# mnastorg/PSI-GNN

Hardware: AMD Instinct MI355X
Metric: fixed-point edges/sec (E' x Broyden iterations/sec) on 1M-node Poisson mesh (higher is better)
Workload: dtype f32

## Files before the change

### psi-gnn_amd/csrc/solver.hip

```cpp
#include "vec_helpers.h"
#include <stdlib.h>
#include <math.h>
#include <algorithm>
#include <vector>

struct Status {
  int32_t n_iter;
  int32_t done;
  int32_t prot_break;
  int32_t stop_reason;
  int32_t lowest_step;
  int32_t cur;
  int32_t low;
  int32_t nxt;
  double lowest_rel, lowest_abs_at;
  double rel0;
  double abs0;
  int32_t lowest_step_abs;
  int32_t stop_abs;
  double s, beta;
};

#define PARTA_LD 32
#define RB 256
#define RA 8
struct psignn_broyden {
  const psignn_plan* plan = nullptr;
  int64_t M = 0;
  int seq_len = D;
  int thr = 0;
  int keep_trace = 0;
  int vec = 16;
  int nblk = 0, npart = 0;
  int vec_ax = 0, nblk_ax = 0;
  int jgroups = 1;
  float* jpart = nullptr;
  float *U = nullptr, *V = nullptr;
  float* xbuf = nullptr;
  float* gbuf[2] = {nullptr, nullptr};
  float *upd = nullptr, *fx = nullptr, *fwork = nullptr;
  float* lwork = nullptr;
  int64_t lwork_floats = 0;
  float* nrm_part = nullptr;
  float* part2 = nullptr;
  int uvu = 0;
  int vec_u = 0, nblk_u = 0, npart_u = 0;
  int u2d_kmax = 0, nblk4 = 0, a_ready = 0;
  int u2d_keep = 0, a_from = 0;
  int u2d_reg = 1;
  float* parta = nullptr;
  int nn_cap = 0;
  float *h0p = nullptr, *prbp = nullptr, *nrmp = nullptr;
  float* part = nullptr;
  int ldp = 0;
  int64_t pstride = 0;
  float* coef = nullptr;
  Status* st = nullptr;
  double *rel_trace = nullptr, *abs_trace = nullptr;
  Status* h_st = nullptr;
  size_t bytes = 0;
  int ext_iter = 0;
  int64_t ld = 0;
  int hist = 0;
  int stop_abs = 0;
  int64_t size_hint = 0;
  int plan_order = 1;
};

__global__ void k_init_status(Status* st, double* rel_trace, double* abs_trace, int thr, int stop_abs = 0) {
  if (threadIdx.x == 0 && blockIdx.x == 0) {
    st->abs0 = 0.0; st->lowest_step_abs = 0; st->stop_abs = stop_abs;
    st->n_iter = 0; st->done = 0; st->prot_break = 0; st->stop_reason = 0; st->lowest_step = 0;
    st->cur = 0; st->low = 0; st->nxt = 1;
    st->lowest_rel = 1e8; st->lowest_abs_at = 1e8; st->rel0 = 0.0; st->s = 0.0; st->beta = 0.0;
  }
  for (int i = blockIdx.x * blockDim.x + threadIdx.x; i < thr; i += gridDim.x * blockDim.x) {
    rel_trace[i] = 0.0;
    abs_trace[i] = 0.0;
  }
}

template <int VEC>
__global__ __launch_bounds__(TB) void k_begin(int64_t M, const float* __restrict__ x0, const float* __restrict__ fx0,
                                              float* __restrict__ xb, float* __restrict__ gx, float* __restrict__ upd) {
  int64_t e0 = elem0<VEC>();
  if (e0 >= M) return;
  float a[VEC], b[VEC];
  ldv<VEC>(x0, e0, M, a);
  ldv<VEC>(fx0, e0, M, b);
  stv<VEC>(xb, e0, M, a);
#pragma unroll
  for (int i = 0; i < VEC; ++i) b[i] -= a[i];
  stv<VEC>(gx, e0, M, b);
  stv<VEC>(upd, e0, M, b);
}

template <int VEC>
__device__ __forceinline__ void xnext_body(int64_t M, const Status* __restrict__ st, float* __restrict__ xb,
                                           const float* __restrict__ upd, float* __restrict__ copy_out) {
  if (st->done) return;
  int64_t e0 = elem0<VEC>();
  if (e0 >= M) return;
  const float* xc = xb + (int64_t)st->cur * M;
  float* xn = xb + (int64_t)st->nxt * M;
  float a[VEC], b[VEC];
  ldv<VEC>(xc, e0, M, a);
  ldv<VEC>(upd, e0, M, b);
#pragma unroll
  for (int i = 0; i < VEC; ++i) a[i] += b[i];
  stv<VEC>(xn, e0, M, a);
  if (copy_out) stv<VEC>(copy_out, e0, M, a);
}
template <int VEC>
__global__ __launch_bounds__(TB) void k_xnext(int64_t M, const Status* __restrict__ st, float* __restrict__ xb,
                                              const float* __restrict__ upd, float* __restrict__ copy_out) {
  xnext_body<VEC>(M, st, xb, upd, copy_out);
}

template <int VEC>
__global__ __launch_bounds__(TB) void k_xtrial(int64_t M, const Status* __restrict__ st, const float* __restrict__ xb,
                                               float* __restrict__ upd, float s, float* __restrict__ out, int commit) {
  if (st->done) return;
  int64_t e0 = elem0<VEC>();
  if (e0 >= M) return;
  const float* xc = xb + (int64_t)st->cur * M;
  float a[VEC], b[VEC];
  ldv<VEC>(xc, e0, M, a);
  ldv<VEC>(upd, e0, M, b);
#pragma unroll
  for (int i = 0; i < VEC; ++i) {
    b[i] *= s;
    a[i] += b[i];
// ... 644 lines not shown
#pragma unroll
        for (int q = 0; q < U2D_UNROLL; ++q) {
          const float cc = __builtin_bit_cast(float, __builtin_amdgcn_readlane(__builtin_bit_cast(int, cv), q));
          const float cb = __builtin_bit_cast(float, __builtin_amdgcn_readlane(__builtin_bit_cast(int, cv), 8 + q));
          a1[0] = fmaf(-cc, u[q].x, a1[0]); a1[1] = fmaf(-cc, u[q].y, a1[1]); a1[2] = fmaf(-cc, u[q].z, a1[2]); a1[3] = fmaf(-cc, u[q].w, a1[3]);
          a2[0] = fmaf(-cb, u[q].x, a2[0]); a2[1] = fmaf(-cb, u[q].y, a2[1]); a2[2] = fmaf(-cb, u[q].z, a2[2]); a2[3] = fmaf(-cb, u[q].w, a2[3]);
        }
      }
      for (; j < j_keep0; ++j) {
        const float cc = rfl(coef[thr + j]), cb = rfl(coef[2 * thr + j]);
        asm volatile("" : "+v"(off));
        const float4 u = ld4_so(U + (int64_t)j * ld, off);
        a1[0] = fmaf(-cc, u.x, a1[0]); a1[1] = fmaf(-cc, u.y, a1[1]); a1[2] = fmaf(-cc, u.z, a1[2]); a1[3] = fmaf(-cc, u.w, a1[3]);
        a2[0] = fmaf(-cb, u.x, a2[0]); a2[1] = fmaf(-cb, u.y, a2[1]); a2[2] = fmaf(-cb, u.z, a2[2]); a2[3] = fmaf(-cb, u.w, a2[3]);
      }
      switch (k - j_keep0) {
        U2R_CASE(KB - 8, false) U2R_CASE(KB - 7, false) U2R_CASE(KB - 6, false) U2R_CASE(KB - 5, false) U2R_CASE(KB - 4, false)
        U2R_CASE(KB - 3, false) U2R_CASE(KB - 2, false) U2R_CASE(KB - 1, false) U2R_CASE(KB, false)
        default: break;
      }
    }
#undef U2R_CASE
  } else {
    const bool in = e0 < M;
    float a1[4] = {0.f, 0.f, 0.f, 0.f}, a2[4] = {0.f, 0.f, 0.f, 0.f};
    if (in) {
      float dg[4];
      ldv<4>(upd, e0, M, a1);
      ldv<4>(dgv, e0, M, dg);
      ldv<4>(gv, e0, M, a2);
#pragma unroll
      for (int i = 0; i < 4; ++i) dg[i] = a2[i] - dg[i];
#pragma unroll
      for (int i = 0; i < 4; ++i) a1[i] = a1[i] + dg[i];
    }
    for (int j = 0; j < k; ++j) {
      float u[4] = {0.f, 0.f, 0.f, 0.f};
      const float cc = coef[thr + j], cb = coef[2 * thr + j];
      if (in) ldv<4>(U + (int64_t)j * ld, e0, M, u);
#pragma unroll
      for (int i = 0; i < 4; ++i) {
        a1[i] = fmaf(-cc, u[i], a1[i]);
        a2[i] = fmaf(-cb, u[i], a2[i]);
      }
    }
    if (in) {
      const float sv = (float)st->s, beta = (float)st->beta;
#pragma unroll
      for (int i = 0; i < 4; ++i) {
        float q = a1[i] / sv;
        q = (q != q) ? 0.f : q;
        a1[i] = q;
        a2[i] = fmaf(-q, beta, a2[i]);
      }
      stv<4>(U + (int64_t)k * ld, e0, M, a1);
      stv<4>(upd, e0, M, a2);
#pragma unroll
      for (int i = 0; i < 4; ++i)
        if (e0 + i >= M) a1[i] = a2[i] = 0.f;
    }
    for (int jj = j_keep0; jj <= k; ++jj) {
      float u[4] = {a1[0], a1[1], a1[2], a1[3]};
      if (jj < k) {
        u[0] = u[1] = u[2] = u[3] = 0.f;
        if (in) ldv<4>(U + (int64_t)jj * ld, e0, M, u);
      }
      float sa = fmaf(u[0], a2[0], fmaf(u[1], a2[1], fmaf(u[2], a2[2], u[3] * a2[3])));
      sa = wave_sum(sa);
      if (lead) ua[wv][jj - j_keep0] = sa;
    }
  }
  __syncthreads();
  if (tid <= k - j_keep0) part[(int64_t)blockIdx.x * PARTA_LD + tid] = (ua[0][tid] + ua[1][tid]) + (ua[2][tid] + ua[3][tid]);
}
template <int KB> struct U2RWaves { static constexpr int value = KB <= 8 ? 8 : KB <= 16 ? 5 : 4; };
template <int KB>
__global__ __launch_bounds__(TB, U2RWaves<KB>::value) void k_sweep_u2r(int64_t M, int k, const Status* __restrict__ st, float* __restrict__ U,
                                                                      float* __restrict__ upd, const float* __restrict__ dgv,
                                                                      const float* __restrict__ gv, const float* __restrict__ coef, int thr,
                                                                      float* __restrict__ part, int64_t ld, int j_keep0) {
  sweep_u2r_body<KB>(M, k, st, U, upd, dgv, gv, coef, thr, part, ld, j_keep0);
}

template <int VEC>
__device__ __forceinline__ void axpy_finish(int64_t M, int k, int64_t e0, float* av, float* a1, float* a2, const float* dg,
                                            const float* g, float* __restrict__ U, float* __restrict__ V,
                                            float* __restrict__ upd, float& p1, float& p2, int64_t ld) {
#pragma unroll
  for (int i = 0; i < VEC; ++i) {
    p1 = fmaf(av[i], dg[i], p1);
    av[i] = (av[i] != av[i]) ? 0.f : av[i];
    p2 = fmaf(av[i], g[i], p2);
  }
  stv<VEC>(V + (int64_t)k * ld, e0, M, av);
  stv<VEC>(U + (int64_t)k * ld, e0, M, a1);
  stv<VEC>(upd, e0, M, a2);
}

template <int VEC>
__device__ __forceinline__ void axpy_body(int64_t M, int k, const Status* __restrict__ st, float* __restrict__ U,
                                             float* __restrict__ V, float* __restrict__ upd ,
                                             const float* __restrict__ dgv, const float* __restrict__ gv,
                                             const float* __restrict__ coef, int thr, float* __restrict__ part, int npart,
                                             int jstride, float* __restrict__ jpart, int64_t ld, const bool split) {
  if (st->done) return;
  const int j0 = blockIdx.y * jstride, j1 = min(k, j0 + jstride);
  int64_t e0 = elem0<VEC>();
  float p1 = 0.f, p2 = 0.f;
  if (e0 < M) {
    float av[VEC], a1[VEC], a2[VEC], dg[VEC], g[VEC];
    if (!split) {
      ldv<VEC>(upd, e0, M, av);
      ldv<VEC>(dgv, e0, M, dg);
      ldv<VEC>(gv, e0, M, g);
#pragma unroll
      for (int i = 0; i < VEC; ++i) dg[i] = g[i] - dg[i];
#pragma unroll
      for (int i = 0; i < VEC; ++i) {
        a1[i] = av[i] + dg[i];
        a2[i] = g[i];
        av[i] = -av[i];
      }
    } else {
#pragma unroll
      for (int i = 0; i < VEC; ++i) av[i] = a1[i] = a2[i] = 0.f;
    }
    for (int j = j0; j < j1; ++j) {
      float u[VEC], v[VEC];
      float ca = coef[j], cc = coef[thr + j], cb = coef[2 * thr + j];
      ldv_stream<VEC>(U + (int64_t)j * ld, e0, M, u);
      ldv_stream<VEC>(V + (int64_t)j * ld, e0, M, v);
#pragma unroll
      for (int i = 0; i < VEC; ++i) {
        av[i] = fmaf(ca, v[i], av[i]);
        a1[i] = fmaf(-cc, u[i], a1[i]);
        a2[i] = fmaf(-cb, u[i], a2[i]);
      }
    }
    if (split) {
      float* base = jpart + (int64_t)blockIdx.y * 3 * M;
      stv<VEC>(base, e0, M, av);
      stv<VEC>(base + M, e0, M, a1);
      stv<VEC>(base + 2 * M, e0, M, a2);
      return;
    }
    axpy_finish<VEC>(M, k, e0, av, a1, a2, dg, g, U, V, upd, p1, p2, ld);
  }
  if (split) return;
  block_pair_store(p1, p2, part, npart);
}
template <int VEC>
__global__ __launch_bounds__(TB) void k_axpy(int64_t M, int k, const Status* __restrict__ st, float* __restrict__ U,
                                             float* __restrict__ V, float* __restrict__ upd ,
                                             const float* __restrict__ dgv, const float* __restrict__ gv,
                                             const float* __restrict__ coef, int thr, float* __restrict__ part, int npart,
                                             int jstride, float* __restrict__ jpart, int64_t ld) {
  axpy_body<VEC>(M, k, st, U, V, upd, dgv, gv, coef, thr, part, npart, jstride, jpart, ld, gridDim.y > 1);
}

template <int VEC>
__device__ __forceinline__ void axpy_combine_body(int64_t M, int k, int G, const Status* __restrict__ st,
                                                     const float* __restrict__ jpart, float* __restrict__ U,
                                                     float* __restrict__ V, float* __restrict__ upd,
                                                     const float* __restrict__ dgv, const float* __restrict__ gv,
                                                     float* __restrict__ part, int npart, int64_t ld) {
  if (st->done) return;
// ... 74 lines not shown

template <int VEC>
__global__ __launch_bounds__(TB) void k_copy_sel(int64_t M, const float* __restrict__ xb, const int32_t* __restrict__ sel,
                                                 int fixed, float* __restrict__ dst) {
  int64_t e0 = elem0<VEC>();
  if (e0 >= M) return;
  int idx = sel ? *sel : fixed;
  float a[VEC];
  ldv<VEC>(xb + (int64_t)idx * M, e0, M, a);
  stv<VEC>(dst, e0, M, a);
}

int psignn_f_eval_p(const psignn_plan_t* p, const float* W, int nl, const float* hbase, const int32_t* d_sel,
                    int64_t stride, const float* h0, const float* prb, const float* nrm, float* out, float* work,
                    hipStream_t st);

int psignn_f_tile_fused(const psignn_plan* p, const float* W, int nl, float* xbuf, int64_t M, const int32_t* st_words,
                        int off_done, int off_cur, int off_nxt, const float* upd, float* gnew,
                        const float* h0, const float* prb, const float* nrm, float* part, hipStream_t st);

#define U2R_KB_MAX 24
#define U2D_LDS_KMAX (PARTA_LD - 1)
static_assert(U2R_KB_MAX + 1 <= PARTA_LD, "the register fold's kept pairs must fit a partials row");
__global__ __launch_bounds__(TB) void kb_sweep_u2d(const BatchDesc* __restrict__ descs, int k, int j_keep0, int par);
static bool u2d_lds_attr(int dev) {
  static int state[64] = {0};
  if (dev < 0 || dev >= 64) return false;
  if (state[dev] == 0) {
    const int want = U2D_LDS_KMAX * TB * 16;
    const bool ok = hipFuncSetAttribute((const void*)k_sweep_u2d, hipFuncAttributeMaxDynamicSharedMemorySize, want) == hipSuccess &&
                    hipFuncSetAttribute((const void*)kb_sweep_u2d, hipFuncAttributeMaxDynamicSharedMemorySize, want) == hipSuccess;
    if (!ok) (void)hipGetLastError();
    state[dev] = ok ? 1 : -1;
  }
  return state[dev] > 0;
}

static int broyden_alloc(psignn_broyden* s) {
  size_t M = (size_t)s->M, thr = (size_t)s->thr;
  const int64_t vec16_min = [] {
    const char* e = getenv("PSIGNN_VEC16_MIN");
    return e ? (int64_t)atoll(e) : (int64_t)3 << 18;
  }();
  const int64_t eff = std::max<int64_t>(s->M, s->size_hint);
  s->vec = eff >= vec16_min ? 16 : 4;
  s->nblk = (int)cdiv(s->M, (int64_t)s->vec * TB);
  const int64_t eff_blk = cdiv(eff, (int64_t)s->vec * TB);
  s->jgroups = eff_blk >= 768 ? 1 : (int)std::min<int64_t>(8, cdiv(768, eff_blk));
  const bool short_shard = s->size_hint > s->M && s->vec == 16 && s->nblk < 512;
  if (short_shard) s->jgroups = 4;
  if (const char* e = getenv("PSIGNN_JGROUPS")) s->jgroups = std::max(1, std::min(8, atoi(e)));
  s->npart = s->nblk * (TB / 64);
  s->vec_ax = s->vec;
  s->nblk_ax = s->nblk;
  const char* e_ax = getenv("PSIGNN_VEC_AX4");
  if (e_ax ? (atoi(e_ax) != 0 && s->vec == 16)
           : (s->vec == 16 && s->jgroups > 1 && (short_shard || cdiv(s->M, (int64_t)4 * TB) >= 512))) {
    s->vec_ax = 4;
    s->nblk_ax = (int)cdiv(s->M, (int64_t)4 * TB);
  }
  s->uvu = 0;
  if (s->vec == 16 && s->jgroups == 1 && s->vec_ax == 16) {
    s->uvu = 1; s->vec_u = 16; s->nblk_u = s->nblk;
  } else if (s->vec_ax == 4 && s->vec == 16) {
    s->uvu = 1; s->vec_u = 4; s->nblk_u = s->nblk_ax;
  }
  if (const char* e = getenv("PSIGNN_UVU")) if (atoi(e) == 0) s->uvu = 0;
  if (s->hist) {
    s->uvu = 1;
    s->vec_u = (s->vec == 16 && s->jgroups == 1 && s->vec_ax == 16) ? 16 : 4;
    s->nblk_u = (int)cdiv(s->M, (int64_t)s->vec_u * TB);
  }
  s->npart_u = s->nblk_u * (TB / 64);
  s->nblk4 = (int)cdiv(s->M, (int64_t)4 * TB);
  const bool fold_ok = s->uvu != 0;
  s->u2d_reg = cdiv(eff, (int64_t)4 * TB) >= 2048 && s->M < ((int64_t)1 << 30);
  if (const char* e = getenv("PSIGNN_U2D_FORM")) s->u2d_reg = ((e[0] == 'l' || e[0] == 'L') ? 0 : 1) && s->M < ((int64_t)1 << 30);
  const int kmax_cap = s->u2d_reg ? U2R_KB_MAX : U2D_LDS_KMAX;
  s->u2d_kmax = fold_ok ? 24 : 0;
  if (const char* e = getenv("PSIGNN_U2D_KMAX")) s->u2d_kmax = fold_ok ? std::max(0, std::min(kmax_cap, atoi(e))) : 0;
  s->u2d_keep = s->u2d_kmax > 0 ? 16 : 0;
  if (const char* e = getenv("PSIGNN_U2D_KEEP")) s->u2d_keep = s->u2d_kmax > 0 ? std::max(0, std::min(s->u2d_kmax, atoi(e))) : 0;
  if (s->hist) s->u2d_kmax = s->u2d_keep = 0;
  if (s->u2d_kmax > 0 && !s->u2d_reg) {
    int dev = 0;
    (void)hipGetDevice(&dev);
    if (!u2d_lds_attr(dev)) {
      s->u2d_kmax = std::min(s->u2d_kmax, 15);
      s->u2d_keep = std::min(s->u2d_keep, 15);
    }
  }
  s->nn_cap = std::max<int>(std::max(s->nblk, s->nblk_ax), s->plan ? (int)s->plan->n_tiles : 0);
  s->ldp = (s->thr + 63) / 64 * 64;
  s->pstride = (int64_t)std::max(std::max(s->nblk, s->nblk_u), std::max(s->nblk_ax, 1)) * s->ldp;
  size_t nx = s->keep_trace ? thr + 2 : 3;
  s->ld = s->hist ? (s->M + 127) / 128 * 128 : (s->M + 63) / 64 * 64;
  size_t ld = (size_t)s->ld;
  const size_t pb = s->hist ? 2 : 4;
  struct { void** p; size_t n; } allocs[] = {
      {(void**)&s->U, thr * ld * pb},  {(void**)&s->V, thr * ld * pb},   {(void**)&s->xbuf, nx * M * 4},
      {(void**)&s->gbuf[0], M * 4},   {(void**)&s->gbuf[1], M * 4},   {(void**)&s->upd, M * 4},
      {(void**)&s->fx, M * 4},        {(void**)&s->part, 3 * (size_t)s->pstride * 4 + 16}, {(void**)&s->parta, (size_t)s->nblk4 * PARTA_LD * 4 + 16},
      {(void**)&s->coef, (3 + RA) * thr * 4 + 16}, {(void**)&s->st, sizeof(Status)},
      {(void**)&s->nrm_part, 2 * (size_t)s->nn_cap * 4 + 16}, {(void**)&s->part2, 2 * (size_t)std::max(s->nblk, s->nblk_u) * 4 + 16},
      {(void**)&s->rel_trace, thr * 8 + 8}, {(void**)&s->abs_trace, thr * 8 + 8}};
  for (auto& a : allocs) {
    if (hipMalloc(a.p, a.n ? a.n : 16) != hipSuccess) {
      psignn_set_error("broyden: hipMalloc of %zu bytes failed (U+V need 2*thr*N*d*4 bytes)", a.n);
      return PSIGNN_ENOMEM;
    }
    s->bytes += a.n;
  }
  if (s->jgroups > 1 && s->vec_ax == s->vec) {
    size_t jb = (size_t)s->jgroups * 3 * M * 4;
    if (hipMalloc((void**)&s->jpart, jb) != hipSuccess) {
      psignn_set_error("broyden: hipMalloc of the split-sweep scratch failed");
      return PSIGNN_ENOMEM;
    }
    s->bytes += jb;
  }
  if (s->plan) {
    size_t wf = (size_t)psignn_f_workspace_floats(s->plan) * 4;
    if (hipMalloc((void**)&s->fwork, wf) != hipSuccess) {
      psignn_set_error("broyden: hipMalloc of f workspace failed");
      return PSIGNN_ENOMEM;
    }
    s->bytes += wf;
    size_t N = (size_t)s->plan->N;
    if (hipMalloc((void**)&s->h0p, M * 4) != hipSuccess || hipMalloc((void**)&s->prbp, N * 3 * 4) != hipSuccess ||
        hipMalloc((void**)&s->nrmp, N * 2 * 4) != hipSuccess) {
      psignn_set_error("broyden: hipMalloc of plan-order inputs failed");
      return PSIGNN_ENOMEM;
    }
    s->bytes += M * 4 + N * 20;
  }
  if (hipHostMalloc((void**)&s->h_st, sizeof(Status)) != hipSuccess) {
    psignn_set_error("broyden: hipHostMalloc failed");
    return PSIGNN_ENOMEM;
  }
  return 0;
}

extern "C" void psignn_broyden_destroy(psignn_broyden_t* s) {
  if (!s) return;
  void* ptrs[] = {s->U, s->V, s->xbuf, s->gbuf[0], s->gbuf[1], s->upd, s->fx, s->fwork, s->part, s->coef, s->st, s->nrm_part, s->part2, s->parta,
                  s->rel_trace, s->abs_trace, s->h0p, s->prbp, s->nrmp, s->jpart, s->lwork};
  for (void* q : ptrs)
    if (q) (void)hipFree(q);
  if (s->h_st) (void)hipHostFree(s->h_st);
  delete s;
}

extern "C" int psignn_broyden_create_opts(psignn_broyden_t** out, const psignn_plan_t* plan, int64_t n_elems, int seq_len, int threshold,
                                          int keep_trace, int64_t shard_elems, int history) {
  ARG_CHECK(out, "out is NULL");
  *out = nullptr;
  ARG_CHECK(history == 0 || history == 1, "history: 0 = fp32 pairs, 1 = bf16 pairs");
  if (plan) {
    ARG_CHECK(threshold > 0 && shard_elems >= 0, "bad arguments");
    ARG_CHECK((n_elems == 0 || n_elems == plan->N * D) && (seq_len == 0 || seq_len == D), "n_elems / seq_len do not match the plan");
  } else {
    ARG_CHECK(n_elems > 0 && threshold > 0 && seq_len > 0 && shard_elems >= 0, "bad sizes");
    ARG_CHECK(cdiv(n_elems, 16 * TB) * (TB / 64) < (int64_t)INT32_MAX, "vector too long");
  }
  psignn_broyden* s = new psignn_broyden();
  s->size_hint = shard_elems;
  s->plan = plan;
  s->M = plan ? plan->N * D : n_elems;
  s->seq_len = plan ? D : seq_len;
  s->thr = threshold;
  s->keep_trace = keep_trace;
  s->hist = history;
  int rc = broyden_alloc(s);
  if (rc) {
    psignn_broyden_destroy(s);
    return rc;
  }
  *out = s;
  return PSIGNN_OK;
}

extern "C" int psignn_broyden_create_n(psignn_broyden_t** out, int64_t n_elems, int seq_len, int threshold, int keep_trace) {
  return psignn_broyden_create_opts(out, nullptr, n_elems, seq_len, threshold, keep_trace, 0, 0);
}

extern "C" int psignn_broyden_create(psignn_broyden_t** out, const psignn_plan_t* plan, int threshold, int keep_trace) {
  return psignn_broyden_create_opts(out, plan, 0, 0, threshold, keep_trace, 0, 0);
}
extern "C" int psignn_broyden_create_for_batch(psignn_broyden_t** out, const psignn_plan_t* plan, int threshold, int keep_trace,
                                               int64_t shard_elems) {
  ARG_CHECK(out, "out is NULL");
  *out = nullptr;
  ARG_CHECK(plan, "bad arguments");
  return psignn_broyden_create_opts(out, plan, 0, 0, threshold, keep_trace, shard_elems, 0);
}

extern "C" size_t psignn_broyden_bytes(const psignn_broyden_t* s) { return s ? s->bytes : 0; }

extern "C" int psignn_broyden_set_stop_mode(psignn_broyden_t* s, int abs_mode) {
  ARG_CHECK(s, "NULL solver");
  s->stop_abs = abs_mode ? 1 : 0;
  return PSIGNN_OK;
}

static inline int sel_off_cur() { return offsetof(Status, cur) / 4; }
static inline int sel_off_low() { return offsetof(Status, low) / 4; }
static inline int sel_off_nxt() { return offsetof(Status, nxt) / 4; }

static inline __bf16* bf16_pairs(float* p) { return reinterpret_cast<__bf16*>(p); }

template <class Target>
static void update_chain(Target& t, int k, double eps) {
  const psignn_broyden& c = t.size_class();
  const int thr = c.thr;
  const int64_t vb = t.vec_bytes();
  const int64_t pe = vb / 4 * t.pair_elem_bytes();
  const int kd = k >= thr ? 0 : k;
  const bool last = k + 1 >= thr;
  if (c.uvu) {
    if (k == 0) t.a_ready() = 0;
    const int a_from = t.a_ready() ? t.a_from() : kd;
    const int n1 = std::min(a_from, kd);
    if (n1 > 0) {
      PROF_BYTES(n1 * pe + vb);
      t.sweep_u1(n1);
    }
    t.reduce_a_check(kd, eps, a_from);
    t.a_ready() = 0;
    if (k >= thr) return;
    PROF_BYTES(last ? 0 : (k + 1) * pe + 3 * vb);
    t.sweep_v(k);
    t.reduce_cb(k);
    const int keep0 = k <= c.u2d_kmax ? 0 : k - c.u2d_keep;
    if (c.u2d_kmax > 0 && (k <= c.u2d_kmax || c.u2d_keep > 0) && !last) {
      PROF_BYTES((k + 1) * pe + 4 * vb);
      const int nk = k - keep0;
      if (!c.u2d_reg) t.sweep_u2d(k, keep0, (size_t)std::max(nk, 1) * TB * 16);
      else if (nk <= 8) t.template sweep_u2r<8>(k, keep0);
      else if (nk <= 16) t.template sweep_u2r<16>(k, keep0);
      else t.template sweep_u2r<24>(k, keep0);
      t.a_ready() = 1;
      t.a_from() = keep0;
    } else {
      PROF_BYTES(last ? 0 : (k + 1) * pe + 4 * vb);
      t.sweep_u2(k);
    }
    return;
  }
  const int G = t.groups(k);
  if (kd > 0) {
    PROF_BYTES((2 * kd + 3) * vb);
    t.dots(kd, G);
  }
  t.reduce_check(kd, eps);
  if (k >= thr) return;
  const bool own_width = c.vec_ax != c.vec;
  const int Ga = own_width ? 1 : G;
  PROF_BYTES(last ? 0 : (2 * k + (Ga > 1 ? 3 * Ga : 6)) * vb);
  t.axpy(k, Ga, own_width);
  if (!own_width && t.combine_due(k, G)) {
    PROF_BYTES(last || G <= 1 ? 0 : (3 * G + 6) * vb);
    t.combine(k, G);
  }
  PROF_BYTES(last ? 0 : 4 * vb);
  t.final_pass(k, own_width);
}

struct SingleTarget {
  psignn_broyden* s;
  hipStream_t st;
  float* gnew;
  const float* gold;
  int np;
  const psignn_broyden& size_class() const { return *s; }
  int64_t vec_bytes() const { return s->M * 4; }
  int pair_elem_bytes() const { return s->hist ? 2 : 4; }
  int& a_ready() { return s->a_ready; }
  int& a_from() { return s->a_from; }
  int groups(int k) const { return (s->jgroups > 1 && k >= 4 * s->jgroups) ? s->jgroups : 1; }
  bool combine_due(int, int G) const { return G > 1; }
  unsigned gu() const { return (unsigned)s->nblk_u; }

  void sweep_u1(int n1) {
    if (s->hist) VLAUNCH("k_sweep_u1_bf16", st, s->vec_u, k_sweep_u1_bf16, (gu(), TB, 0, st), s->M, n1, s->st, bf16_pairs(s->U), s->upd, s->part, s->ldp, s->ld);
    else VLAUNCH("k_sweep_u1", st, s->vec_u, k_sweep_u1, (gu(), TB, 0, st), s->M, n1, s->st, s->U, s->upd, s->part, s->ldp, s->ld);
  }
  void reduce_a_check(int kd, double eps, int a_from) {
    LAUNCH("k_reduce_check", st, (k_reduce_a_check<<<dim3(std::max(kd, 1), RA + 1), RB, 0, st>>>(
        s->st, s->part, s->nblk_u, s->ldp, s->thr, kd, s->coef, s->nrm_part, np, s->rel_trace, s->abs_trace, eps, s->seq_len, s->keep_trace,
        s->parta, s->nblk4, a_from)));
  }
  void sweep_v(int k) {
    if (s->hist) VLAUNCH("k_sweep_v_bf16", st, s->vec_u, k_sweep_v_bf16, (gu(), TB, 0, st), s->M, k, s->st, bf16_pairs(s->V), s->upd, gold, gnew, s->coef, s->part, s->pstride, s->ldp, s->part2, s->nblk_u, s->ld, s->thr);
    else VLAUNCH("k_sweep_v", st, s->vec_u, k_sweep_v, (gu(), TB, 0, st), s->M, k, s->st, s->V, s->upd, gold, gnew, s->coef, s->part, s->pstride, s->ldp, s->part2, s->nblk_u, s->ld, s->thr);
  }
  void reduce_cb(int k) {
    LAUNCH("k_reduce_cb", st, (k_reduce_cb<<<dim3(std::max(k, 1), 3), RB, 0, st>>>(s->st, s->part, s->nblk_u, s->pstride, s->ldp, s->thr, k, s->coef, s->part2, s->nblk_u)));
  }
  template <int KB>
  void sweep_u2r(int k, int keep0) {
    LAUNCH("k_sweep_u2d", st, (k_sweep_u2r<KB><<<(unsigned)s->nblk4, TB, 0, st>>>(s->M, k, s->st, s->U, s->upd, gold, gnew, s->coef, s->thr, s->parta, s->ld, keep0)));
  }
  void sweep_u2d(int k, int keep0, size_t lds) {
    LAUNCH("k_sweep_u2d", st, (k_sweep_u2d<<<(unsigned)s->nblk4, TB, lds, st>>>(s->M, k, s->st, s->U, s->upd, gold, gnew, s->coef, s->thr, s->parta, s->ld, keep0)));
  }
  void sweep_u2(int k) {
    if (s->hist) VLAUNCH("k_sweep_u2_bf16", st, s->vec_u, k_sweep_u2_bf16, (gu(), TB, 0, st), s->M, k, s->st, bf16_pairs(s->U), s->upd, gold, gnew, s->coef, s->thr, s->ld);
    else VLAUNCH("k_sweep_u2", st, s->vec_u, k_sweep_u2, (gu(), TB, 0, st), s->M, k, s->st, s->U, s->upd, gold, gnew, s->coef, s->thr, s->ld);
  }
  void dots(int kd, int G) {
    VLAUNCH("k_dots", st, s->vec, k_dots, (dim3((unsigned)s->nblk, G), TB, 0, st), s->M, kd, s->st, s->U, s->V, s->upd, gold, gnew, s->part, s->pstride, s->ldp, (int)cdiv(kd, G), s->ld);
  }
  void reduce_check(int kd, double eps) {
    LAUNCH("k_reduce_check", st, (k_reduce_check<<<dim3(std::max(kd, 1), 4), RB, 0, st>>>(
        s->st, s->part, s->nblk, s->pstride, s->ldp, s->thr, kd, s->coef, s->nrm_part, np, s->rel_trace, s->abs_trace, eps, s->seq_len, s->keep_trace)));
  }
  void axpy(int k, int G, bool own_width) {
    const int nb = own_width ? s->nblk_ax : s->nblk;
    VLAUNCH("k_axpy", st, own_width ? s->vec_ax : s->vec, k_axpy, (dim3((unsigned)nb, G), TB, 0, st), s->M, k, s->st, s->U, s->V, s->upd, gold, gnew, s->coef, s->thr, s->part, nb, (int)cdiv(std::max(k, 1), G), s->jpart, s->ld);
  }
  void combine(int k, int G) {
    VLAUNCH("k_axpy_combine", st, s->vec, k_axpy_combine, ((unsigned)s->nblk, TB, 0, st), s->M, k, G, s->st, s->jpart, s->U, s->V, s->upd, gold, gnew, s->part, s->nblk, s->ld);
  }
  void final_pass(int k, bool own_width) {
    const int nb = own_width ? s->nblk_ax : s->nblk;
    VLAUNCH("k_final", st, own_width ? s->vec_ax : s->vec, k_final, ((unsigned)nb, TB, 0, st), s->M, k, s->st, s->U, s->upd, s->ld, s->part, nb);
  }
};

static void launch_update(psignn_broyden* s, int k, double eps, hipStream_t st, int fused_npart = 0) {
  SingleTarget t{s, st, s->gbuf[(k + 1) & 1], s->gbuf[k & 1], fused_npart ? fused_npart : s->nblk};
  if (!fused_npart) {
    PROF_BYTES(3 * (int64_t)s->M * 4);
    VLAUNCH("k_resid", st, s->vec, k_resid, ((unsigned)s->nblk, TB, 0, st), s->M, s->st, s->xbuf, s->fx, t.gnew, s->nrm_part, s->nblk);
  }
  update_chain(t, k, eps);
}

static int read_status(psignn_broyden* s, hipStream_t st) {
  HIP_TRY(hipMemcpyAsync(s->h_st, s->st, sizeof(Status), hipMemcpyDeviceToHost, st));
  HIP_TRY(hipStreamSynchronize(st));
  return 0;
}

static int finish(psignn_broyden* s, float* d_result, psignn_solve_info_t* info, double* h_rel, double* h_abs,
                  hipStream_t st) {
  unsigned g = (unsigned)s->nblk;
  int rc = 0;
  if (d_result) {
    const int32_t* sel_low = reinterpret_cast<const int32_t*>(s->st) + sel_off_low();
    if (s->plan && s->plan_order) {
      VPLAIN(s->vec, k_copy_sel, (g, TB, 0, st), s->M, s->xbuf, sel_low, 0, s->fx);
      if ((rc = psignn_plan_permute(s->plan, s->fx, D, d_result, 0, st))) return rc;
    } else {
      VPLAIN(s->vec, k_copy_sel, (g, TB, 0, st), s->M, s->xbuf, sel_low, 0, d_result);
    }
  }
  if ((rc = read_status(s, st))) return rc;
  const Status& h = *s->h_st;
  if (info) {
    info->nstep = h.stop_abs ? h.lowest_step_abs : h.lowest_step;
    info->n_iter = h.n_iter;
    info->prot_break = h.prot_break;
    info->stop_reason = h.stop_reason;
    info->lowest = h.lowest_rel;
    info->lowest_abs = h.lowest_abs_at;
  }
  int n = h.n_iter;
  if (h_rel && n > 0) HIP_TRY(hipMemcpy(h_rel, s->rel_trace, (size_t)n * 8, hipMemcpyDeviceToHost));
  if (h_abs && n > 0) HIP_TRY(hipMemcpy(h_abs, s->abs_trace, (size_t)n * 8, hipMemcpyDeviceToHost));
  for (int i = n; i < s->thr; ++i) {
    if (h_rel) h_rel[i] = h.lowest_rel;
    if (h_abs) h_abs[i] = h.lowest_abs_at;
  }
  HIP_TRY(hipGetLastError());
  return PSIGNN_OK;
}

extern "C" int psignn_broyden_solve(psignn_broyden_t* s, const float* W, int nl, const float* h0, const float* prb,
                                    const float* nrm, double eps, int poll_every, float* d_result,
                                    psignn_solve_info_t* info, double* h_rel, double* h_abs, void* stream) {
  ARG_CHECK(s && s->plan, "solver was not created from a mesh plan");
  ARG_CHECK(W && h0 && prb, "NULL argument");
  ARG_CHECK(!s->plan->mixed || nrm, "mixed plan needs unit normals");
// ... 55 lines not shown
  __shared__ double sh[RB];
  const BatchDesc& d = descs[blockIdx.z];
  reduce_check_body(reinterpret_cast<Status*>(d.st), d.part, d.nblk, d.pstride, (d.thr + 63) / 64 * 64, d.thr, k, d.coef, d.nrm_part, d.n_nrm, d.rel_trace,
                    d.abs_trace, eps, d.seq_len, d.keep_trace, sh);
}
template <int VEC>
__global__ __launch_bounds__(TB) void kb_axpy(const BatchDesc* __restrict__ descs, int k, int own_width, int par) {
  const BatchDesc& d = descs[blockIdx.z];
  const int G = own_width ? 1 : batch_groups(d, k);
  const int nb = own_width ? d.nblk_ax : d.nblk;
  if ((int)blockIdx.x >= nb || (int)blockIdx.y >= G) return;
  axpy_body<VEC>(d.M, k, reinterpret_cast<const Status*>(d.st), d.U, d.V, d.upd, bd_gold(d, par), bd_gnew(d, par), d.coef, d.thr, d.part, nb,
                 idiv_up(k > 1 ? k : 1, G), d.jpart, d.ld, G > 1);
}
template <int VEC>
__global__ __launch_bounds__(TB) void kb_axpy_combine(const BatchDesc* __restrict__ descs, int k, int par) {
  const BatchDesc& d = descs[blockIdx.z];
  const int G = batch_groups(d, k);
  if ((int)blockIdx.x >= d.nblk || G <= 1) return;
  axpy_combine_body<VEC>(d.M, k, G, reinterpret_cast<const Status*>(d.st), d.jpart, d.U, d.V, d.upd, bd_gold(d, par), bd_gnew(d, par), d.part, d.nblk, d.ld);
}
template <int VEC>
__global__ __launch_bounds__(TB) void kb_final(const BatchDesc* __restrict__ descs, int k, int own_width) {
  __shared__ double sh[TB];
  const BatchDesc& d = descs[blockIdx.z];
  const int nb = own_width ? d.nblk_ax : d.nblk;
  if ((int)blockIdx.x >= nb) return;
  final_body<VEC>(d.M, k, reinterpret_cast<Status*>(d.st), d.U, d.upd, d.ld, d.part, nb, sh);
}
template <int VEC>
__global__ __launch_bounds__(TB) void kb_sweep_u1(const BatchDesc* __restrict__ descs, int k) {
  const BatchDesc& d = descs[blockIdx.z];
  if ((int)blockIdx.x >= d.nblk_u) return;
  sweep_u1_body<VEC>(d.M, k, reinterpret_cast<const Status*>(d.st), d.U, d.upd, d.part, (d.thr + 63) / 64 * 64, d.ld);
}
__global__ __launch_bounds__(RB) void kb_reduce_a_check(const BatchDesc* __restrict__ descs, int k, double eps, int a_from) {
  __shared__ double sh[RB];
  const BatchDesc& d = descs[blockIdx.z];
  reduce_a_check_body(reinterpret_cast<Status*>(d.st), d.part, d.nblk_u, (d.thr + 63) / 64 * 64, d.thr, k, d.coef, d.nrm_part, d.n_nrm, d.rel_trace,
                      d.abs_trace, eps, d.seq_len, d.keep_trace, sh, d.parta, d.nblk4, a_from);
}
__global__ __launch_bounds__(TB) void kb_sweep_u2d(const BatchDesc* __restrict__ descs, int k, int j_keep0, int par) {
  const BatchDesc& d = descs[blockIdx.z];
  if ((int)blockIdx.x >= d.nblk4) return;
  sweep_u2d_body(d.M, k, reinterpret_cast<const Status*>(d.st), d.U, d.upd, bd_gold(d, par), bd_gnew(d, par), d.coef, d.thr, d.parta, d.ld, j_keep0);
}
template <int KB>
__global__ __launch_bounds__(TB, U2RWaves<KB>::value) void kb_sweep_u2r(const BatchDesc* __restrict__ descs, int k, int j_keep0, int par) {
  const BatchDesc& d = descs[blockIdx.z];
  if ((int)blockIdx.x >= d.nblk4) return;
  sweep_u2r_body<KB>(d.M, k, reinterpret_cast<const Status*>(d.st), d.U, d.upd, bd_gold(d, par), bd_gnew(d, par), d.coef, d.thr, d.parta, d.ld, j_keep0);
}
template <int VEC>
__global__ __launch_bounds__(TB) void kb_sweep_v(const BatchDesc* __restrict__ descs, int k, int par) {
  const BatchDesc& d = descs[blockIdx.z];
  if ((int)blockIdx.x >= d.nblk_u) return;
  sweep_v_body<VEC>(d.M, k, reinterpret_cast<const Status*>(d.st), d.V, d.upd, bd_gold(d, par), bd_gnew(d, par), d.coef, d.part, d.pstride, (d.thr + 63) / 64 * 64, d.part2,
                    d.nblk_u, d.ld, d.thr);
}
__global__ __launch_bounds__(RB) void kb_reduce_cb(const BatchDesc* __restrict__ descs, int k) {
  __shared__ double sh[RB];
  const BatchDesc& d = descs[blockIdx.z];
  reduce_cb_body(reinterpret_cast<Status*>(d.st), d.part, d.nblk_u, d.pstride, (d.thr + 63) / 64 * 64, d.thr, k, d.coef, d.part2, d.nblk_u, sh);
}
template <int VEC>
__global__ __launch_bounds__(TB) void kb_sweep_u2(const BatchDesc* __restrict__ descs, int k, int par) {
  const BatchDesc& d = descs[blockIdx.z];
  if ((int)blockIdx.x >= d.nblk_u) return;
  sweep_u2_body<VEC>(d.M, k, reinterpret_cast<const Status*>(d.st), d.U, d.upd, bd_gold(d, par), bd_gnew(d, par), d.coef, d.thr, d.ld);
}
__global__ void kb_all_done(const BatchDesc* __restrict__ descs, int n, int off_done, int32_t* __restrict__ all_done) {
  if (threadIdx.x == 0 && blockIdx.x == 0) {
    int a = 1;
    for (int m = 0; m < n; ++m) a &= descs[m].st[off_done] != 0;
    *all_done = a;
  }
}

struct BatchShape {
  int n = 0, max_g = 0, max_ga = 0, max_gu = 0, max_g4 = 0, max_G = 1;
  int64_t Mtot4 = 0;
  int a_ready = 0;
  int a_from_next = 0;
};
static BatchShape shard_shape(int n, psignn_broyden_t* const* sv) {
  BatchShape sh;
  sh.n = n;
  for (int m = 0; m < n; ++m) {
    const psignn_broyden* s = sv[m];
    sh.max_g = std::max(sh.max_g, s->nblk);
    sh.max_ga = std::max(sh.max_ga, s->nblk_ax);
    sh.max_gu = std::max(sh.max_gu, s->nblk_u);
    sh.max_g4 = std::max(sh.max_g4, s->nblk4);
    sh.max_G = std::max(sh.max_G, s->jgroups);
    sh.Mtot4 += s->M * 4;
  }
  return sh;
}

struct ShardTarget {
  const psignn_broyden* s0;
  BatchShape& sh;
  const BatchDesc* dd;
  hipStream_t st;
  const psignn_broyden& size_class() const { return *s0; }
  int64_t vec_bytes() const { return sh.Mtot4; }
  int pair_elem_bytes() const { return 4; }
  int& a_ready() { return sh.a_ready; }
  int& a_from() { return sh.a_from_next; }
  int groups(int k) const { return (sh.max_G > 1 && k >= 4 * sh.max_G) ? sh.max_G : 1; }
  bool combine_due(int k, int) const { return sh.max_G > 1 && k >= 4 * 2; }
  dim3 grid(int x, int y = 1) const { return dim3((unsigned)x, (unsigned)y, (unsigned)sh.n); }

  void sweep_u1(int n1) { VLAUNCH("k_sweep_u1", st, s0->vec_u, kb_sweep_u1, (grid(sh.max_gu), TB, 0, st), dd, n1); }
  void reduce_a_check(int kd, double eps, int a_from) {
    LAUNCH("k_reduce_check", st, (kb_reduce_a_check<<<grid(std::max(kd, 1), RA + 1), RB, 0, st>>>(dd, kd, eps, a_from)));
  }
  void sweep_v(int k) { VLAUNCH("k_sweep_v", st, s0->vec_u, kb_sweep_v, (grid(sh.max_gu), TB, 0, st), dd, k, k & 1); }
  void reduce_cb(int k) { LAUNCH("k_reduce_cb", st, (kb_reduce_cb<<<grid(std::max(k, 1), 3), RB, 0, st>>>(dd, k))); }
  template <int KB>
  void sweep_u2r(int k, int keep0) { LAUNCH("k_sweep_u2d", st, (kb_sweep_u2r<KB><<<grid(sh.max_g4), TB, 0, st>>>(dd, k, keep0, k & 1))); }
  void sweep_u2d(int k, int keep0, size_t lds) { LAUNCH("k_sweep_u2d", st, (kb_sweep_u2d<<<grid(sh.max_g4), TB, lds, st>>>(dd, k, keep0, k & 1))); }
  void sweep_u2(int k) { VLAUNCH("k_sweep_u2", st, s0->vec_u, kb_sweep_u2, (grid(sh.max_gu), TB, 0, st), dd, k, k & 1); }
  void dots(int kd, int) { VLAUNCH("k_dots", st, s0->vec, kb_dots, (grid(sh.max_g, sh.max_G), TB, 0, st), dd, kd, kd & 1); }
  void reduce_check(int kd, double eps) { LAUNCH("k_reduce_check", st, (kb_reduce_check<<<grid(std::max(kd, 1), 4), RB, 0, st>>>(dd, kd, eps))); }
  void axpy(int k, int, bool own_width) {
    if (own_width) VLAUNCH("k_axpy", st, s0->vec_ax, kb_axpy, (grid(sh.max_ga), TB, 0, st), dd, k, 1, k & 1);
    else VLAUNCH("k_axpy", st, s0->vec, kb_axpy, (grid(sh.max_g, sh.max_G), TB, 0, st), dd, k, 0, k & 1);
  }
  void combine(int k, int) { VLAUNCH("k_axpy_combine", st, s0->vec, kb_axpy_combine, (grid(sh.max_g), TB, 0, st), dd, k, k & 1); }
  void final_pass(int k, bool own_width) {
    VLAUNCH("k_final", st, own_width ? s0->vec_ax : s0->vec, kb_final, (grid(own_width ? sh.max_ga : sh.max_g), TB, 0, st), dd, k, own_width ? 1 : 0);
  }
};

static void fill_desc(const psignn_broyden* s, BatchDesc& d) {
  d.M = s->M; d.ld = s->ld; d.nblk = s->nblk; d.npart = s->npart; d.nblk_ax = s->nblk_ax; d.jgroups = s->jgroups;
  d.thr = s->thr; d.seq_len = s->seq_len; d.keep_trace = s->keep_trace; d.n_tiles = (int)s->plan->n_tiles;
  d.st = reinterpret_cast<int32_t*>(s->st);
  d.U = s->U; d.V = s->V; d.xbuf = s->xbuf; d.g0 = s->gbuf[0]; d.g1 = s->gbuf[1]; d.upd = s->upd; d.part = s->part; d.coef = s->coef;
  d.nrm_part = s->nrm_part; d.jpart = s->jpart; d.rel_trace = s->rel_trace; d.abs_trace = s->abs_trace;
  d.ctx = s->plan->d_ctx; d.h0p = s->h0p; d.prbp = s->prbp;
  d.part2 = s->part2; d.nblk_u = s->nblk_u; d.npart_u = s->npart_u;
  d.parta = s->parta; d.nblk4 = s->nblk4; d.pad_ = 0; d.pstride = s->pstride;
  d.fx = s->fx; d.xcopy = s->h0p; d.pad2_ = 0;
}
static int shard_all_done(const BatchDesc* d_descs, int n, int32_t* d_done, int32_t* h_done, hipStream_t st) {
  kb_all_done<<<1, 64, 0, st>>>(d_descs, n, offsetof(Status, done) / 4, d_done);
  HIP_TRY(hipMemcpyAsync(h_done, d_done, 4, hipMemcpyDeviceToHost, st));
  HIP_TRY(hipStreamSynchronize(st));
  return PSIGNN_OK;
}
static int shard_finish(int n, psignn_broyden_t** sv, float* const* d_results, psignn_solve_info_t* infos, double* const* h_rel,
                        double* const* h_abs, hipStream_t st) {
  int rc = PSIGNN_OK;
  for (int m = 0; m < n && rc == PSIGNN_OK; ++m)
    rc = finish(sv[m], d_results ? d_results[m] : nullptr, infos ? &infos[m] : nullptr, h_rel ? h_rel[m] : nullptr,
                h_abs ? h_abs[m] : nullptr, st);
  return rc;
}

int psignn_f_tile_fused_batch(const BatchDesc* d_descs, int n_mesh, int n_slots, int max_rows, const float* W, int mixed,
                              int off_done, int off_cur, int off_nxt, int par, hipStream_t st);

static bool same_size_class(const psignn_broyden* a, const psignn_broyden* b) {
  return a->vec == b->vec && a->vec_ax == b->vec_ax && a->uvu == b->uvu && a->vec_u == b->vec_u && a->thr == b->thr &&
         a->u2d_kmax == b->u2d_kmax && a->u2d_keep == b->u2d_keep && a->u2d_reg == b->u2d_reg;
}

extern "C" int psignn_broyden_batchable(int n, psignn_broyden_t* const* sv) {
  if (n <= 0 || !sv || !sv[0] || !sv[0]->plan) return 0;
  const psignn_broyden* s0 = sv[0];
  for (int m = 0; m < n; ++m) {
    const psignn_broyden* s = sv[m];
    if (!s || !s->plan || !s->plan->tiled || s->plan->mixed != s0->plan->mixed) return 0;
    if (s->hist) return 0;
    if (!same_size_class(s, s0)) return 0;
  }
  return 1;
}

extern "C" int psignn_broyden_solve_batch(int n, psignn_broyden_t** sv, const float* W, int nl, const float* const* h0,
                                          const float* const* prb, const float* const* nrm, double eps, int poll_every,
                                          float* const* d_results, psignn_solve_info_t* infos, double* const* h_rel,
                                          double* const* h_abs, void* stream) {
  ARG_CHECK(n > 0 && sv && W && h0 && prb, "bad arguments");
  ARG_CHECK(nl == 1, "the batched solver runs single-layer blocks");
  ARG_CHECK(psignn_broyden_batchable(n, sv),
            "batched solve: tiled plans of one boundary-condition family and one size class, fp32 pair history (psignn_broyden_batchable)");
  for (int m = 0; m < n; ++m) {
    ARG_CHECK(h0[m] && prb[m], "NULL argument");
    ARG_CHECK(!sv[m]->plan->mixed || (nrm && nrm[m]), "mixed plans need unit normals");
// ... 426 lines not shown
```

Measured before the change: 2.210 billion.

## Fold all history dot products into the u2 sweep for mid-range Broyden iterations

Adds a k_sweep_u2w kernel for iterations 25-48. While it writes the new U column and the update, it also computes every dot product of the update against the history columns. The older columns are reduced through per-thread LDS accumulators and the last 16 through wave reductions into parta. With these results in hand, the next iteration's separate sweep_u1 pass over the older history is skipped, which removes one full read of the U history per iteration. The cost is more registers and LDS per block, a separate kernel instantiation for each k, and lower occupancy through launch bounds of 2-4 waves.

Measured after the change: 2.216 billion (median of 6 runs). Within noise of the previous version (+0.3%).

```diff
diff --git a/psi-gnn_amd/csrc/solver.hip b/psi-gnn_amd/csrc/solver.hip
--- a/psi-gnn_amd/csrc/solver.hip
+++ b/psi-gnn_amd/csrc/solver.hip
@@ -48,6 +48,7 @@
   int u2d_kmax = 0, nblk4 = 0, a_ready = 0;
   int u2d_keep = 0, a_from = 0;
   int u2d_reg = 1;
+  int u2w = 0, a_swept = 0;
   float* parta = nullptr;
   int nn_cap = 0;
   float *h0p = nullptr, *prbp = nullptr, *nrmp = nullptr;
@@ -858,6 +859,166 @@
   sweep_u2r_body<KB>(M, k, st, U, upd, dgv, gv, coef, thr, part, ld, j_keep0);
 }
 
+#define U2W_KEEP 16
+#define U2W_NK_MIN 25
+#define U2W_NK_MAX 48
+static_assert(U2W_KEEP + 1 <= PARTA_LD, "the whole fold's window must fit a partials row");
+template <int NK> struct U2WWaves { static constexpr int value = NK <= 25 ? 4 : NK <= 32 ? 3 : 2; };
+template <int NK>
+__global__ __launch_bounds__(TB, U2WWaves<NK>::value) void k_sweep_u2w(int64_t M, const Status* __restrict__ st, float* __restrict__ U,
+                                                                      float* __restrict__ upd, const float* __restrict__ dgv,
+                                                                      const float* __restrict__ gv, const float* __restrict__ coef, int thr,
+                                                                      float* __restrict__ parta, int nblk4, float* __restrict__ part, int ldp,
+                                                                      int64_t ld) {
+  constexpr int NO = NK - U2W_KEEP;
+  __shared__ float acc[NO][TB];
+  __shared__ float ta[TB / 64][4][U2W_KEEP + 1];
+  __shared__ float so[TB / 64][NO];
+  if (__builtin_amdgcn_readfirstlane(st->done)) return;
+  const int tid = threadIdx.x;
+  const int wv = __builtin_amdgcn_readfirstlane(tid >> 6);
+  const int lane = tid & 63;
+  const bool lead = lane == 0;
+  const int64_t wave_e0 = ((int64_t)blockIdx.x * TB + (int64_t)__builtin_amdgcn_readfirstlane(tid & ~63)) * 16;
+  if (wave_e0 + 1024 <= M) {
+    uint32_t off = ((blockIdx.x * (uint32_t)TB + ((uint32_t)tid & ~63u)) * 16u + ((uint32_t)tid & 63u) * 4u) * 4u;
+    float ccv = 0.f, cbv = 0.f;
+    if (lane < NK) {
+      ccv = coef[thr + lane];
+      cbv = coef[2 * thr + lane];
+    }
+    const float sv = rfl((float)st->s), beta = rfl((float)st->beta);
+#pragma unroll
+    for (int q = 0; q < NO; ++q) acc[q][tid] = 0.f;
+#pragma unroll 1
+    for (int i = 0; i < 4; ++i) {
+      asm volatile("" : "+v"(off));
+      int64_t ldo = ld;
+      asm volatile("" : "+s"(ldo));
+      asm volatile("" : "+v"(ccv), "+v"(cbv));
+      float4 kp[NK];
+#pragma unroll
+      for (int q = 0; q < NK; ++q) kp[q] = ld4_so(U + (int64_t)q * ldo, off);
+      float a1[4], a2[4];
+      {
+        const float4 x = ld4_so(upd, off), go = ld4_so(dgv, off), g = ld4_so(gv, off);
+        a1[0] = x.x + (g.x - go.x); a1[1] = x.y + (g.y - go.y); a1[2] = x.z + (g.z - go.z); a1[3] = x.w + (g.w - go.w);
+        a2[0] = g.x; a2[1] = g.y; a2[2] = g.z; a2[3] = g.w;
+      }
+#pragma unroll
+      for (int q = 0; q < NK; ++q) {
+        if (q > 0 && q % 8 == 0) __builtin_amdgcn_sched_barrier(0);
+        const float cc = __builtin_bit_cast(float, __builtin_amdgcn_readlane(__builtin_bit_cast(int, ccv), q));
+        const float cb = __builtin_bit_cast(float, __builtin_amdgcn_readlane(__builtin_bit_cast(int, cbv), q));
+        a1[0] = fmaf(-cc, kp[q].x, a1[0]); a1[1] = fmaf(-cc, kp[q].y, a1[1]); a1[2] = fmaf(-cc, kp[q].z, a1[2]); a1[3] = fmaf(-cc, kp[q].w, a1[3]);
+        a2[0] = fmaf(-cb, kp[q].x, a2[0]); a2[1] = fmaf(-cb, kp[q].y, a2[1]); a2[2] = fmaf(-cb, kp[q].z, a2[2]); a2[3] = fmaf(-cb, kp[q].w, a2[3]);
+      }
+#pragma unroll
+      for (int c = 0; c < 4; ++c) {
+        float q = a1[c] / sv;
+        q = (q != q) ? 0.f : q;
+        a1[c] = q;
+        a2[c] = fmaf(-q, beta, a2[c]);
+      }
+      st4_so(U + (int64_t)NK * ldo, off, make_float4(a1[0], a1[1], a1[2], a1[3]));
+      st4_so(upd, off, make_float4(a2[0], a2[1], a2[2], a2[3]));
+#pragma unroll
+      for (int q = 0; q < NO; ++q) {
+        float s = acc[q][tid];
+        s = fmaf(a2[0], kp[q].x, s); s = fmaf(a2[1], kp[q].y, s); s = fmaf(a2[2], kp[q].z, s); s = fmaf(a2[3], kp[q].w, s);
+        acc[q][tid] = s;
+      }
+#pragma unroll
+      for (int q = NO; q < NK; ++q) {
+        float sa = fmaf(kp[q].x, a2[0], fmaf(kp[q].y, a2[1], fmaf(kp[q].z, a2[2], kp[q].w * a2[3])));
+        sa = wave_sum(sa);
+        if (lead) ta[wv][i][q - NO] = sa;
+      }
+      float sa = fmaf(a1[0], a2[0], fmaf(a1[1], a2[1], fmaf(a1[2], a2[2], a1[3] * a2[3])));
+      sa = wave_sum(sa);
+      if (lead) ta[wv][i][U2W_KEEP] = sa;
+      off += 1024u;
+    }
+  } else if (wave_e0 < M) {
+#pragma unroll 1
+    for (int q = 0; q < NO; ++q) acc[q][tid] = 0.f;
+#pragma unroll 1
+    for (int i = 0; i < 4; ++i) {
+      const int64_t e0 = wave_e0 + i * 256 + lane * 4;
+      const bool in = e0 < M;
+      float a1[4] = {0.f, 0.f, 0.f, 0.f}, a2[4] = {0.f, 0.f, 0.f, 0.f};
+      if (in) {
+        float dg[4];
+        ldv<4>(upd, e0, M, a1);
+        ldv<4>(dgv, e0, M, dg);
+        ldv<4>(gv, e0, M, a2);
+#pragma unroll
+        for (int c = 0; c < 4; ++c) dg[c] = a2[c] - dg[c];
+#pragma unroll
+        for (int c = 0; c < 4; ++c) a1[c] = a1[c] + dg[c];
+      }
+#pragma unroll 1
+      for (int j = 0; j < NK; ++j) {
+        float u[4] = {0.f, 0.f, 0.f, 0.f};
+        const float cc = coef[thr + j], cb = coef[2 * thr + j];
+        if (in) ldv<4>(U + (int64_t)j * ld, e0, M, u);
+#pragma unroll
+        for (int c = 0; c < 4; ++c) {
+          a1[c] = fmaf(-cc, u[c], a1[c]);
+          a2[c] = fmaf(-cb, u[c], a2[c]);
+        }
+      }
+      if (in) {
+        const float sv = (float)st->s, beta = (float)st->beta;
+#pragma unroll
+        for (int c = 0; c < 4; ++c) {
+          float q = a1[c] / sv;
+          q = (q != q) ? 0.f : q;
+          a1[c] = q;
+          a2[c] = fmaf(-q, beta, a2[c]);
+        }
+        stv<4>(U + (int64_t)NK * ld, e0, M, a1);
+        stv<4>(upd, e0, M, a2);
+#pragma unroll
+        for (int c = 0; c < 4; ++c)
+          if (e0 + c >= M) a1[c] = a2[c] = 0.f;
+      }
+#pragma unroll 1
+      for (int j = 0; j < NO; ++j) {
+        float u[4] = {0.f, 0.f, 0.f, 0.f};
+        if (in) ldv<4>(U + (int64_t)j * ld, e0, M, u);
+        float s = acc[j][tid];
+        s = fmaf(a2[0], u[0], s); s = fmaf(a2[1], u[1], s); s = fmaf(a2[2], u[2], s); s = fmaf(a2[3], u[3], s);
+        acc[j][tid] = s;
+      }
+#pragma unroll 1
+      for (int j = NO; j <= NK; ++j) {
+        float u[4] = {a1[0], a1[1], a1[2], a1[3]};
+        if (j < NK) {
+          u[0] = u[1] = u[2] = u[3] = 0.f;
+          if (in) ldv<4>(U + (int64_t)j * ld, e0, M, u);
+        }
+        float sa = fmaf(u[0], a2[0], fmaf(u[1], a2[1], fmaf(u[2], a2[2], u[3] * a2[3])));
+        sa = wave_sum(sa);
+        if (lead) ta[wv][i][j - NO] = sa;
+      }
+    }
+  }
+  if (wave_e0 < M) {
+#pragma unroll
+    for (int q = 0; q < NO; ++q) {
+      const float s = wave_sum(acc[q][tid]);
+      if (lead) so[wv][q] = s;
+    }
+  } else if (lane < NO) {
+    so[wv][lane] = 0.f;
+  }
+  __syncthreads();
+  if (tid < NO) part[(int64_t)blockIdx.x * ldp + tid] = (so[0][tid] + so[1][tid]) + (so[2][tid] + so[3][tid]);
+  const int64_t row = (int64_t)blockIdx.x * 4 + wv;
+  if (lane <= U2W_KEEP && row < nblk4) parta[row * PARTA_LD + lane] = (ta[wv][0][lane] + ta[wv][1][lane]) + (ta[wv][2][lane] + ta[wv][3][lane]);
+}
+
 template <int VEC>
 __device__ __forceinline__ void axpy_finish(int64_t M, int k, int64_t e0, float* av, float* a1, float* a2, const float* dg,
                                             const float* g, float* __restrict__ U, float* __restrict__ V,
@@ -1098,6 +1259,12 @@
   s->u2d_keep = s->u2d_kmax > 0 ? 16 : 0;
   if (const char* e = getenv("PSIGNN_U2D_KEEP")) s->u2d_keep = s->u2d_kmax > 0 ? std::max(0, std::min(s->u2d_kmax, atoi(e))) : 0;
   if (s->hist) s->u2d_kmax = s->u2d_keep = 0;
+  s->u2w = s->uvu && s->vec_u == 16 && s->jgroups == 1 && !s->hist && s->u2d_reg && s->u2d_keep == U2W_KEEP && s->u2d_kmax == U2W_NK_MIN - 1 &&
+           s->M < ((int64_t)1 << 30);
+  {
+    const char* e = getenv("PSIGNN_U2W");
+    if (e ? atoi(e) == 0 : cdiv(eff, (int64_t)4 * TB) < 2048) s->u2w = 0;
+  }
   if (s->u2d_kmax > 0 && !s->u2d_reg) {
     int dev = 0;
     (void)hipGetDevice(&dev);
@@ -1237,18 +1404,25 @@
     if (k == 0) t.a_ready() = 0;
     const int a_from = t.a_ready() ? t.a_from() : kd;
     const int n1 = std::min(a_from, kd);
-    if (n1 > 0) {
+    if (n1 > 0 && !(t.a_ready() && t.a_swept())) {
       PROF_BYTES(n1 * pe + vb);
       t.sweep_u1(n1);
     }
     t.reduce_a_check(kd, eps, a_from);
     t.a_ready() = 0;
+    t.a_swept() = 0;
     if (k >= thr) return;
     PROF_BYTES(last ? 0 : (k + 1) * pe + 3 * vb);
     t.sweep_v(k);
     t.reduce_cb(k);
     const int keep0 = k <= c.u2d_kmax ? 0 : k - c.u2d_keep;
-    if (c.u2d_kmax > 0 && (k <= c.u2d_kmax || c.u2d_keep > 0) && !last) {
+    if (t.whole_fold(k) && !last) {
+      PROF_BYTES((k + 1) * pe + 4 * vb);
+      t.sweep_u2w(k);
+      t.a_ready() = 1;
+      t.a_from() = k - U2W_KEEP;
+      t.a_swept() = 1;
+    } else if (c.u2d_kmax > 0 && (k <= c.u2d_kmax || c.u2d_keep > 0) && !last) {
       PROF_BYTES((k + 1) * pe + 4 * vb);
       const int nk = k - keep0;
       if (!c.u2d_reg) t.sweep_u2d(k, keep0, (size_t)std::max(nk, 1) * TB * 16);
@@ -1293,6 +1467,8 @@
   int pair_elem_bytes() const { return s->hist ? 2 : 4; }
   int& a_ready() { return s->a_ready; }
   int& a_from() { return s->a_from; }
+  int& a_swept() { return s->a_swept; }
+  bool whole_fold(int k) const { return s->u2w && k >= U2W_NK_MIN && k <= U2W_NK_MAX; }
   int groups(int k) const { return (s->jgroups > 1 && k >= 4 * s->jgroups) ? s->jgroups : 1; }
   bool combine_due(int, int G) const { return G > 1; }
   unsigned gu() const { return (unsigned)s->nblk_u; }
@@ -1316,6 +1492,16 @@
   template <int KB>
   void sweep_u2r(int k, int keep0) {
     LAUNCH("k_sweep_u2d", st, (k_sweep_u2r<KB><<<(unsigned)s->nblk4, TB, 0, st>>>(s->M, k, s->st, s->U, s->upd, gold, gnew, s->coef, s->thr, s->parta, s->ld, keep0)));
+  }
+  void sweep_u2w(int k) {
+#define U2W_CASE(n) case (n): LAUNCH("k_sweep_u2d", st, (k_sweep_u2w<(n)><<<gu(), TB, 0, st>>>(s->M, s->st, s->U, s->upd, gold, gnew, s->coef, s->thr, s->parta, s->nblk4, s->part, s->ldp, s->ld))); break;
+    switch (k) {
+      U2W_CASE(25) U2W_CASE(26) U2W_CASE(27) U2W_CASE(28) U2W_CASE(29) U2W_CASE(30) U2W_CASE(31) U2W_CASE(32)
+      U2W_CASE(33) U2W_CASE(34) U2W_CASE(35) U2W_CASE(36) U2W_CASE(37) U2W_CASE(38) U2W_CASE(39) U2W_CASE(40)
+      U2W_CASE(41) U2W_CASE(42) U2W_CASE(43) U2W_CASE(44) U2W_CASE(45) U2W_CASE(46) U2W_CASE(47) U2W_CASE(48)
+      default: break;
+    }
+#undef U2W_CASE
   }
   void sweep_u2d(int k, int keep0, size_t lds) {
     LAUNCH("k_sweep_u2d", st, (k_sweep_u2d<<<(unsigned)s->nblk4, TB, lds, st>>>(s->M, k, s->st, s->U, s->upd, gold, gnew, s->coef, s->thr, s->parta, s->ld, keep0)));
@@ -1537,6 +1723,7 @@
   int64_t Mtot4 = 0;
   int a_ready = 0;
   int a_from_next = 0;
+  int a_swept = 0;
 };
 static BatchShape shard_shape(int n, psignn_broyden_t* const* sv) {
   BatchShape sh;
@@ -1563,6 +1750,9 @@
   int pair_elem_bytes() const { return 4; }
   int& a_ready() { return sh.a_ready; }
   int& a_from() { return sh.a_from_next; }
+  int& a_swept() { return sh.a_swept; }
+  bool whole_fold(int) const { return false; }
+  void sweep_u2w(int) {}
   int groups(int k) const { return (sh.max_G > 1 && k >= 4 * sh.max_G) ? sh.max_G : 1; }
   bool combine_due(int k, int) const { return sh.max_G > 1 && k >= 4 * 2; }
   dim3 grid(int x, int y = 1) const { return dim3((unsigned)x, (unsigned)y, (unsigned)sh.n); }
```
